# bbc/turingcodec

Hardware: AMD Instinct MI355X
Metric: encoded fps (havoc hot path, primitive-batch throughput: one picture's primitive calls per frame as whole-frame batches; (higher is better)
Workload: dtype u8; 1 GPU; 1920x1080 8-bit 4:2:0 random-access QP32 speed=medium B-frame, MEASURED call mix of the reference encoder on this clip generator (profiles/r04_reference_call_mi; calls_per_frame=3944815, launches_per_frame=49, pictures_in_flight=2, parallelism=single GPU

## Files before the change

### turingcodec_amd/csrc/kernels_metric.hip

```cpp
#include "common.h"

#include <cstdlib>

namespace havoc_gpu {


template <int S>
__device__ __forceinline__ uint32_t sad_dword(uint32_t a, uint32_t b, uint32_t acc)
{
    if (S == 1) return __builtin_amdgcn_sad_u8(a, b, acc);
    return __builtin_amdgcn_sad_u16(a, b, acc);
}

#ifndef SADL
#define SADL 16
#endif
constexpr int kSadLanes = SADL;
__device__ __forceinline__ int sad_group_sum(int v)
{
    v += __builtin_amdgcn_update_dpp(0, v, 0x111, 0xf, 0xf, true);
    v += __builtin_amdgcn_update_dpp(0, v, 0x112, 0xf, 0xf, true);
    v += __builtin_amdgcn_update_dpp(0, v, 0x114, 0xf, 0xe, true);
    if (kSadLanes == 16) v += __builtin_amdgcn_update_dpp(0, v, 0x118, 0xf, 0xc, true);
    return v;
// ... 99 lines not shown
#pragma unroll
    for (int k = 0; k < WAYS; ++k)
    {
        int t = sad_group_sum((int)acc[k]);
        if (S == 2) t >>= 2;
        if (live && lane == kSadLanes - 1) out[job * WAYS + k] = t;
    }
}

constexpr int kSadWinBytes = 1536;

template <int S, int CB>
__device__ __forceinline__ void sad4_window_strips(const char *src, uint32_t s0, uint32_t ssb, const char *ref, uint32_t a0, uint32_t rsb, const __attribute__((address_space(3))) uint32_t *buf_r,
                                                   __attribute__((address_space(3))) uint32_t *buf_w, int pitchD, int chunks, int lead, const int (&ox)[4], const int (&oy)[4],
                                                   int spready, int rowBytes, int h, int hs, int lane, uint32_t (&acc)[4])
{
    const int wstep = smallDiv(kSadLanes, chunks);
    const int wr0 = smallDiv(lane, chunks), wc = lane - mul24(wr0, chunks);
    const bool copies = wr0 < wstep;
    const int cpr = rowBytes / CB;
    const int rpi = smallDiv(kSadLanes, cpr);
    const int y0 = smallDiv(lane, cpr);
    const int xb = (lane - mul24(y0, cpr)) * CB;
    const bool sums = y0 < rpi;
    int lo[4], sh[4];
#pragma unroll
    for (int k = 0; k < 4; ++k)
    {
        const int bo = lead + ox[k] + xb;
        lo[k] = mul24(y0 + oy[k], pitchD) + (bo >> 2);
        sh[k] = bo & 3;
    }
    const int lstep = mul24(rpi, pitchD);
    const uint32_t gstep = mulu24(wstep, rsb), sstep = mulu24(rpi, ssb);
    const int wlstep = mul24(wstep, pitchD);
    for (int ys = 0; ys < h; ys += hs)
    {
        const int he = min(hs, h - ys), nrows = he + spready;
        if (copies)
        {
            uint32_t g = a0 + mulu24(ys + wr0, rsb) + wc * 16;
            int l = mul24(wr0, pitchD) + wc * 4;
            for (int r = wr0; r < nrows; r += wstep, g += gstep, l += wlstep)
            {
                const u32x4 v = ld16(ref + g);
                buf_w[l] = v.x; buf_w[l + 1] = v.y; buf_w[l + 2] = v.z; buf_w[l + 3] = v.w;
            }
        }
        __builtin_amdgcn_fence(__ATOMIC_RELEASE, "wavefront");
        __builtin_amdgcn_wave_barrier();
        __builtin_amdgcn_fence(__ATOMIC_ACQUIRE, "wavefront");
        if (sums)
        {
            uint32_t sp = s0 + mulu24(ys + y0, ssb) + xb;
            int l = 0;
#pragma unroll 2
            for (int y = y0; y < he; y += rpi, sp += sstep, l += lstep)
            {
                if (CB == 16)
                {
                    const u32x4 a = ld16(src + sp);
#pragma unroll
                    for (int k = 0; k < 4; ++k)
                    {
                        const auto q = buf_r + lo[k] + l;
                        const uint32_t d0 = q[0], d1 = q[1], d2 = q[2], d3 = q[3], d4 = q[4];
                        acc[k] = sad_dword<S>(a.x, __builtin_amdgcn_alignbyte(d1, d0, sh[k]), acc[k]);
                        acc[k] = sad_dword<S>(a.y, __builtin_amdgcn_alignbyte(d2, d1, sh[k]), acc[k]);
                        acc[k] = sad_dword<S>(a.z, __builtin_amdgcn_alignbyte(d3, d2, sh[k]), acc[k]);
                        acc[k] = sad_dword<S>(a.w, __builtin_amdgcn_alignbyte(d4, d3, sh[k]), acc[k]);
                    }
                }
                else if (CB == 8)
                {
                    const u32x2 a = ld8(src + sp);
#pragma unroll
                    for (int k = 0; k < 4; ++k)
                    {
                        const auto q = buf_r + lo[k] + l;
                        const uint32_t d0 = q[0], d1 = q[1], d2 = q[2];
                        acc[k] = sad_dword<S>(a.x, __builtin_amdgcn_alignbyte(d1, d0, sh[k]), acc[k]);
                        acc[k] = sad_dword<S>(a.y, __builtin_amdgcn_alignbyte(d2, d1, sh[k]), acc[k]);
                    }
                }
                else
                {
                    const uint32_t a = ld4(src + sp);
#pragma unroll
                    for (int k = 0; k < 4; ++k)
                    {
                        const auto q = buf_r + lo[k] + l;
                        acc[k] = sad_dword<S>(a, __builtin_amdgcn_alignbyte(q[1], q[0], sh[k]), acc[k]);
                    }
                }
            }
        }
        __builtin_amdgcn_fence(__ATOMIC_RELEASE, "wavefront");
        __builtin_amdgcn_wave_barrier();
    }
}

template <int S, int WB>
__device__ __forceinline__ void sad4_job(const char *__restrict__ src, long stride_src, const char *__restrict__ ref, long stride_ref, float inv_stride_ref,
                                         const int32_t *__restrict__ j, bool live, uint32_t *gbuf, int lane, int (&total)[4])
{
    const int so = j[0], w = j[5], h = live ? j[6] : 0;
    int ro[4];
#pragma unroll
    for (int k = 0; k < 4; ++k) ro[k] = j[1 + k];
    const long ssb = stride_src * S, rsb = stride_ref * S;
    const char *s = src + (long)so * S;
    uint32_t acc[4] = {0, 0, 0, 0};
    const int rowBytes = w * S;

    int dx[4] = {0, 0, 0, 0}, dy[4] = {0, 0, 0, 0};
    const int st = (int)stride_ref, half = st >> 1;
#pragma unroll
    for (int k = 1; k < 4; ++k)
    {
        const int delta = ro[k] - ro[0];
        int q = (int)floorf(((float)delta + (float)half) * inv_stride_ref);
        int r = delta - q * st;
        if (r < -half) { --q; r += st; }
        if (r >= st - half) { ++q; r -= st; }
        dx[k] = r; dy[k] = q;
    }
    const int mindx = min(min(dx[0], dx[1]), min(dx[2], dx[3])), maxdx = max(max(dx[0], dx[1]), max(dx[2], dx[3]));
    const int mindy = min(min(dy[0], dy[1]), min(dy[2], dy[3])), maxdy = max(max(dy[0], dy[1]), max(dy[2], dy[3]));
    const int spready = maxdy - mindy;
    const long minoff = ((long)ro[0] + mul24(mindy, st) + mindx) * S;
    const int lead = (int)(reinterpret_cast<uintptr_t>(ref + minoff) & 15);
    const int chunks = (lead + rowBytes + (maxdx - mindx) * S + 15) >> 4;
    const int pitchD = 4 * chunks + 1;
    const int fit = chunks > 0 && chunks <= kSadLanes ? smallDiv(WB * S / 4, pitchD) - spready : 0;
    const bool chunked = (rowBytes & 15) == 0 ? rowBytes <= 16 * kSadLanes : (rowBytes & 7) == 0 ? rowBytes <= 8 * kSadLanes : (rowBytes & 3) == 0 && rowBytes <= 4 * kSadLanes;
    const bool rows24 = (unsigned)spready < 1024u && (unsigned)h <= 64u && ssb < (1 << 23);
    const bool near = rows24 && minoff + (long)mulu24(h + spready, (uint32_t)rsb) + 16 * chunks < (1ll << 32) && ((long)so * S + (long)mulu24(h, (uint32_t)ssb) + rowBytes) < (1ll << 32);
    const bool window = live && chunked && chunks <= kSadLanes && minoff >= 16 && fit >= min(h, 4) && fit >= 1 && near;
    if (window)
    {
        int ox[4], oy[4];
#pragma unroll
        for (int k = 0; k < 4; ++k)
        {
            ox[k] = (dx[k] - mindx) * S;
            oy[k] = dy[k] - mindy;
        }
        const uint32_t a0 = (uint32_t)(minoff - lead), s0 = (uint32_t)so * S;
        const auto buf_r = (const __attribute__((address_space(3))) uint32_t *)(gbuf);
        const auto buf_w = (__attribute__((address_space(3))) uint32_t *)(gbuf);
        const int hs = min(fit, h);
        if ((rowBytes & 15) == 0) sad4_window_strips<S, 16>(src, s0, (uint32_t)ssb, ref, a0, (uint32_t)rsb, buf_r, buf_w, pitchD, chunks, lead, ox, oy, spready, rowBytes, h, hs, lane, acc);
        else if ((rowBytes & 7) == 0) sad4_window_strips<S, 8>(src, s0, (uint32_t)ssb, ref, a0, (uint32_t)rsb, buf_r, buf_w, pitchD, chunks, lead, ox, oy, spready, rowBytes, h, hs, lane, acc);
        else sad4_window_strips<S, 4>(src, s0, (uint32_t)ssb, ref, a0, (uint32_t)rsb, buf_r, buf_w, pitchD, chunks, lead, ox, oy, spready, rowBytes, h, hs, lane, acc);
    }
    else
    {
        typedef typename Sample<S>::T T;
        const char *r[4];
#pragma unroll
        for (int k = 0; k < 4; ++k) r[k] = ref + (long)ro[k] * S;
        if ((rowBytes & 15) == 0 && rowBytes <= 16 * kSadLanes) sad_block<S, 4, 16, 1>(s, ssb, r, rsb, rowBytes, h, lane, acc);
        else if ((rowBytes & 7) == 0 && rowBytes <= 8 * kSadLanes) sad_block<S, 4, 8, 1>(s, ssb, r, rsb, rowBytes, h, lane, acc);
        else if ((rowBytes & 3) == 0 && rowBytes <= 4 * kSadLanes) sad_block<S, 4, 4, 1>(s, ssb, r, rsb, rowBytes, h, lane, acc);
        else
        {
            const FastDiv fd(w);
            for (int i = lane; i < w * h; i += kSadLanes)
            {
                const int y = fd.div(i), x = i - y * w;
                const int a = reinterpret_cast<const T *>(s + y * ssb)[x];
#pragma unroll
                for (int k = 0; k < 4; ++k) acc[k] += abs(a - (int)reinterpret_cast<const T *>(r[k] + y * rsb)[x]);
            }
        }
    }
#pragma unroll
    for (int k = 0; k < 4; ++k)
    {
        int t = sad_group_sum((int)acc[k]);
        if (S == 2) t >>= 2;
        total[k] = t;
    }
}

template <int S, int WB = kSadWinBytes, int MINW = 1>
__global__ __launch_bounds__(256, MINW) void k_sad4w(const char *__restrict__ src, long stride_src, const char *__restrict__ ref, long stride_ref, float inv_stride_ref,
                                               const int32_t *__restrict__ jobs, int njobs, int32_t *__restrict__ out)
{
    constexpr int kBufD = WB * S / 4 + 16;
    __shared__ uint32_t lds[(256 / kSadLanes) * kBufD + 4];
    const int group = threadIdx.x / kSadLanes, lane = threadIdx.x & (kSadLanes - 1);
    const int job = xcd_block(blockIdx.x, gridDim.x) * (256 / kSadLanes) + group;
    const bool live = job < njobs;
    int total[4];
    sad4_job<S, WB>(src, stride_src, ref, stride_ref, inv_stride_ref, jobs + (long)(live ? job : 0) * 8, live, &lds[group * kBufD], lane, total);
    if (live && lane == kSadLanes - 1)
#pragma unroll
        for (int k = 0; k < 4; ++k) out[job * 4 + k] = total[k];
}

constexpr int kRunMax = 128;

template <int S, int CB, int U>
__device__ __forceinline__ void sad4_run_calls(const __attribute__((address_space(3))) uint32_t *win, const __attribute__((address_space(3))) uint32_t *srcw,
                                               const __attribute__((address_space(3))) uint32_t *cand, int pitchD, int lead, int mndx, int mndy, int rowBytes, int h,
                                               int count, int group, int ngroups, int lane, int32_t *__restrict__ out)
{
    const int cpr = rowBytes / CB;
    const int rpi = smallDiv(kSadLanes, cpr);
    const int y0 = smallDiv(lane, cpr);
    const int xb = (lane - mul24(y0, cpr)) * CB;
    const bool sums = y0 < rpi;
    const int lstep = mul24(rpi, pitchD);
    const int s0 = (mul24(y0, rowBytes) + xb) >> 2, sstep = mul24(rpi, rowBytes) >> 2;
    const int base = lead + xb - mndx * S;
    for (int c0 = group; c0 < count; c0 += ngroups * U)
    {
        int lo[4 * U], sh[4 * U];
        uint32_t acc[4 * U];
#pragma unroll
        for (int u = 0; u < U; ++u)
        {
            const int c = min(c0 + u * ngroups, count - 1);
            uint32_t v4[4];
            if (true)
            {
                const u32x4 cv = *reinterpret_cast<const __attribute__((address_space(3))) u32x4 *>(cand + 4 * c);
                v4[0] = cv.x; v4[1] = cv.y; v4[2] = cv.z; v4[3] = cv.w;
            }
#pragma unroll
            for (int k = 0; k < 4; ++k)
            {
                const int v = (int)v4[k];
                const int dx = (int)(short)(v & 0xffff), dy = v >> 16;
                const int bo = base + dx * S;
                lo[4 * u + k] = mul24(y0 + dy - mndy, pitchD) + (bo >> 2);
                sh[4 * u + k] = bo & 3;
                acc[4 * u + k] = 0;
            }
        }
        if (sums)
        {
            int l = 0, sp = s0;
#pragma unroll 2
            for (int y = y0; y < h; y += rpi, sp += sstep, l += lstep)
            {
                if (CB == 16)
                {
                    const u32x4 av = *reinterpret_cast<const __attribute__((address_space(3))) u32x4 *>(srcw + sp);
#pragma unroll
                    for (int k = 0; k < 4 * U; ++k)
                    {
                        const auto q = win + lo[k] + l;
                        const uint32_t d0 = q[0], d1 = q[1], d2 = q[2], d3 = q[3], d4 = q[4];
                        acc[k] = sad_dword<S>(av.x, __builtin_amdgcn_alignbyte(d1, d0, sh[k]), acc[k]);
                        acc[k] = sad_dword<S>(av.y, __builtin_amdgcn_alignbyte(d2, d1, sh[k]), acc[k]);
                        acc[k] = sad_dword<S>(av.z, __builtin_amdgcn_alignbyte(d3, d2, sh[k]), acc[k]);
                        acc[k] = sad_dword<S>(av.w, __builtin_amdgcn_alignbyte(d4, d3, sh[k]), acc[k]);
                    }
                }
                else if (CB == 8)
                {
                    const u32x2 av = *reinterpret_cast<const __attribute__((address_space(3))) u32x2 *>(srcw + sp);
#pragma unroll
                    for (int k = 0; k < 4 * U; ++k)
                    {
                        const auto q = win + lo[k] + l;
                        const uint32_t d0 = q[0], d1 = q[1], d2 = q[2];
                        acc[k] = sad_dword<S>(av.x, __builtin_amdgcn_alignbyte(d1, d0, sh[k]), acc[k]);
                        acc[k] = sad_dword<S>(av.y, __builtin_amdgcn_alignbyte(d2, d1, sh[k]), acc[k]);
                    }
                }
                else
                {
                    const uint32_t a0 = srcw[sp];
#pragma unroll
                    for (int k = 0; k < 4 * U; ++k)
                    {
                        const auto q = win + lo[k] + l;
                        acc[k] = sad_dword<S>(a0, __builtin_amdgcn_alignbyte(q[1], q[0], sh[k]), acc[k]);
                    }
                }
            }
        }
#pragma unroll
        for (int u = 0; u < U; ++u)
        {
            const int c = c0 + u * ngroups;
#pragma unroll
            for (int k = 0; k < 4; ++k)
            {
                int t = sad_group_sum((int)acc[4 * u + k]);
                if (S == 2) t >>= 2;
                if (lane == kSadLanes - 1 && c < count) out[4 * c + k] = t;
            }
        }
    }
}

typedef u32x4 __attribute__((aligned(4))) u32x4_dw;
typedef u32x2 __attribute__((aligned(4))) u32x2_dw;

template <int S, int ND, bool SG>
__device__ __forceinline__ uint32_t sad_lane_rows(const __attribute__((address_space(3))) uint32_t *q, const __attribute__((address_space(3))) uint32_t *s, int pitchD,
                                                  int nd, int rows, int sh, const uint32_t *__restrict__ gs, int gpitch)
{
    uint32_t acc = 0;
    if (SG)
    {
        if (ND >= 4)
        {
            uint32_t a1 = 0, a2 = 0, a3 = 0;
#pragma unroll 2
            for (int y = 0; y < rows; ++y, q += pitchD, gs += gpitch)
            {
                uint32_t prev = q[0];
#pragma unroll
                for (int i = 0; i < ND; i += 4)
                {
                    const u32x4 a = *reinterpret_cast<const u32x4_dw *>(gs + i);
                    const uint32_t d1 = q[i + 1], d2 = q[i + 2], d3 = q[i + 3], d4 = q[i + 4];
                    acc = sad_dword<S>(a.x, __builtin_amdgcn_alignbyte(d1, prev, sh), acc);
                    a1 = sad_dword<S>(a.y, __builtin_amdgcn_alignbyte(d2, d1, sh), a1);
                    a2 = sad_dword<S>(a.z, __builtin_amdgcn_alignbyte(d3, d2, sh), a2);
                    a3 = sad_dword<S>(a.w, __builtin_amdgcn_alignbyte(d4, d3, sh), a3);
                    prev = d4;
                }
            }
            acc += a1 + a2 + a3;
        }
        else if (ND == 2)
        {
#pragma unroll 4
            for (int y = 0; y < rows; ++y, q += pitchD, gs += gpitch)
            {
                const u32x2 a = *reinterpret_cast<const u32x2_dw *>(gs);
                const uint32_t d0 = q[0], d1 = q[1], d2 = q[2];
                acc = sad_dword<S>(a.x, __builtin_amdgcn_alignbyte(d1, d0, sh), acc);
                acc = sad_dword<S>(a.y, __builtin_amdgcn_alignbyte(d2, d1, sh), acc);
            }
        }
        else
        {
            for (int y = 0; y < rows; ++y, q += pitchD, gs += gpitch)
            {
                uint32_t prev = q[0];
                for (int i = 0; i < nd; ++i)
                {
                    const uint32_t d = q[i + 1];
                    acc = sad_dword<S>(gs[i], __builtin_amdgcn_alignbyte(d, prev, sh), acc);
                    prev = d;
                }
            }
        }
        return acc;
    }
    if (ND >= 4)
    {
#pragma unroll 2
        for (int y = 0; y < rows; ++y, q += pitchD, s += ND)
        {
            uint32_t prev = q[0];
#pragma unroll
            for (int i = 0; i < ND; i += 4)
            {
                const u32x4 a = *reinterpret_cast<const __attribute__((address_space(3))) u32x4 *>(s + i);
                const uint32_t d1 = q[i + 1], d2 = q[i + 2], d3 = q[i + 3], d4 = q[i + 4];
                acc = sad_dword<S>(a.x, __builtin_amdgcn_alignbyte(d1, prev, sh), acc);
                acc = sad_dword<S>(a.y, __builtin_amdgcn_alignbyte(d2, d1, sh), acc);
                acc = sad_dword<S>(a.z, __builtin_amdgcn_alignbyte(d3, d2, sh), acc);
                acc = sad_dword<S>(a.w, __builtin_amdgcn_alignbyte(d4, d3, sh), acc);
                prev = d4;
            }
        }
    }
    else if (ND == 2)
    {
#pragma unroll 4
        for (int y = 0; y < rows; ++y, q += pitchD, s += 2)
        {
            const u32x2 a = *reinterpret_cast<const __attribute__((address_space(3))) u32x2 *>(s);
            const uint32_t d0 = q[0], d1 = q[1], d2 = q[2];
            acc = sad_dword<S>(a.x, __builtin_amdgcn_alignbyte(d1, d0, sh), acc);
            acc = sad_dword<S>(a.y, __builtin_amdgcn_alignbyte(d2, d1, sh), acc);
        }
    }
    else
    {
        for (int y = 0; y < rows; ++y, q += pitchD, s += nd)
        {
            uint32_t prev = q[0];
            for (int i = 0; i < nd; ++i)
            {
                const uint32_t d = q[i + 1];
                acc = sad_dword<S>(s[i], __builtin_amdgcn_alignbyte(d, prev, sh), acc);
                prev = d;
            }
        }
    }
    return acc;
}

template <int S, int NW, bool SG>
__device__ __forceinline__ void sad4_run_lanes(const __attribute__((address_space(3))) uint32_t *win, const __attribute__((address_space(3))) uint32_t *srcw,
                                               const __attribute__((address_space(3))) uint32_t *cand, uint32_t *s_acc, int pitchD, int lead, int mndx,
                                               int mndy, int rowBytes, int h, int count, int tid, int32_t *__restrict__ out, const uint32_t *__restrict__ gsrc, int gpitch)
{
    const int P = 4 * count, nd = rowBytes >> 2, chunks = (P + 63) >> 6;
    const int wave = __builtin_amdgcn_readfirstlane(tid >> 6), lane = tid & 63;
    int ns = 1;
    while (ns < 8 && chunks * ns < NW && h >= 16 * ns) ns *= 2;
    const int rps = (h + ns - 1) / ns;
    if (ns > 1)
    {
        for (int i = tid; i < P; i += 64 * NW) s_acc[i] = 0;
        __syncthreads();
    }
    for (int t = wave; t < chunks * ns; t += NW)
    {
        const int chunk = ns == 1 ? t : t / ns, slice = t - chunk * ns;
        const int pos = chunk * 64 + lane;
        const int p = pos;
        const int v = (int)cand[min(p, P - 1)];
        const int col = (int)(short)(v & 0xffff) - mndx, row = (v >> 16) - mndy;
        const int bo = lead + col * S, sh = bo & 3;
        const int yBeg = slice * rps, rows = min(h, yBeg + rps) - yBeg;
        const auto q = win + mul24(row + yBeg, pitchD) + (bo >> 2);
        const auto sp = srcw + yBeg * nd;
        const uint32_t *gs = gsrc + (long)yBeg * gpitch;
        uint32_t acc;
        if (S == 2 && nd == 32) acc = sad_lane_rows<S, 32, SG>(q, sp, pitchD, nd, rows, sh, gs, gpitch);
        else if (nd == 16) acc = sad_lane_rows<S, 16, SG>(q, sp, pitchD, nd, rows, sh, gs, gpitch);
        else if (nd == 8) acc = sad_lane_rows<S, 8, SG>(q, sp, pitchD, nd, rows, sh, gs, gpitch);
        else if (nd == 4) acc = sad_lane_rows<S, 4, SG>(q, sp, pitchD, nd, rows, sh, gs, gpitch);
        else if (nd == 2) acc = sad_lane_rows<S, 2, SG>(q, sp, pitchD, nd, rows, sh, gs, gpitch);
        else acc = sad_lane_rows<S, 0, SG>(q, sp, pitchD, nd, rows, sh, gs, gpitch);
        if (p < P)
        {
            if (ns == 1) out[p] = (int32_t)(S == 2 ? acc >> 2 : acc);
            else atomicAdd(&s_acc[p], acc);
        }
    }
    if (ns > 1)
    {
        __syncthreads();
        for (int p = tid; p < P; p += 64 * NW) out[p] = (int32_t)(S == 2 ? s_acc[p] >> 2 : s_acc[p]);
    }
}

template <int S>
struct RunLds
{
    static constexpr int kWinD = (S == 1 ? 16 : 32) * 256;
    static constexpr int kSrcD = 64 * 64 * S / 4;
    __attribute__((aligned(16))) uint32_t lds[kWinD + kSrcD + 8];
    __attribute__((aligned(16))) uint32_t cand[kRunMax * 4];
    uint32_t acc[kRunMax * 4];
    int box[6];
};

template <int S, int NW, int U, bool SRCG>
__device__ __forceinline__ void sad4_run_general(RunLds<S> &sh, const char *__restrict__ src, long stride_src, const char *__restrict__ ref, long stride_ref,
                                                 float inv_stride_ref, const int32_t *__restrict__ jobs, int njobs, const int32_t *__restrict__ runs, int run,
                                                 int32_t *__restrict__ out)
{
    constexpr int T = 64 * NW, NG = T / kSadLanes;
    constexpr int kWinD = RunLds<S>::kWinD, kSrcD = RunLds<S>::kSrcD;
    constexpr int kFallWB = 1024, kFallD = kFallWB * S / 4 + 16;
    static_assert(NG * kFallD + 4 <= kWinD + kSrcD, "the call-by-call path's buffers must fit the run's LDS");
    uint32_t (&lds)[kWinD + kSrcD + 8] = sh.lds;
    uint32_t (&s_cand)[kRunMax * 4] = sh.cand;
    uint32_t (&s_acc)[kRunMax * 4] = sh.acc;
    int (&s_box)[6] = sh.box;
    const int tid = threadIdx.x, lane = tid & (kSadLanes - 1), group = tid / kSadLanes;
    const int32_t *rr = runs + (long)run * 8;
    const int first = rr[0], count = rr[1], boxOff = rr[2], boxW = rr[3], boxH = rr[4];
    if (first < 0 || count <= 0 || (long)first + count > njobs) return;
    const int32_t *j0 = jobs + (long)first * 8;
    const int so = j0[0], ro0 = j0[1], w = j0[5], h = j0[6];
    const int st = (int)stride_ref, half = st >> 1;
    const int rowBytes = w * S;
    const long ssb = stride_src * S, rsb = stride_ref * S;
    const bool chunked = (rowBytes & 15) == 0 ? rowBytes <= 16 * kSadLanes : (rowBytes & 7) == 0 ? rowBytes <= 8 * kSadLanes : (rowBytes & 3) == 0 && rowBytes <= 4 * kSadLanes;
    const bool srcScalar = U == 0 && SRCG && (((reinterpret_cast<uintptr_t>(src) + (long)so * S) | ssb) & 3) == 0;
    const bool given = boxW > 0 && boxH > 0 && boxW < st;
    int mndx = 0, mndy = 0, spanx, spready, ok = count <= kRunMax;
    long minoff;
    if (given)
    {
        spanx = boxW - w;
        spready = boxH - h;
        minoff = (long)boxOff * S;
        ok &= spanx >= 0 && spready >= 0 && boxOff >= 0;
    }
    else
    {
        if (tid < 6) s_box[tid] = tid == 4 ? 1 : 0;
        __syncthreads();
        int mn_x = 0, mx_x = 0, mn_y = 0, mx_y = 0;
        for (int p = tid; p < 4 * min(count, kRunMax); p += T)
        {
            const int32_t *j = j0 + (p >> 2) * 8;
            const int delta = j[1 + (p & 3)] - ro0;
            int q = (int)floorf(((float)delta + (float)half) * inv_stride_ref);
            long rl = (long)delta - (long)q * st;
            if (rl < -half) { --q; rl += st; }
            if (rl >= st - half) { ++q; rl -= st; }
            ok &= (j[0] == so) & (j[5] == w) & (j[6] == h) & (q >= -32768) & (q < 32768) & (rl >= -32768) & (rl < 32768);
            const int r = (int)rl;
            s_cand[p] = (uint32_t)(r & 0xffff) | ((uint32_t)q << 16);
            mn_x = min(mn_x, r); mx_x = max(mx_x, r); mn_y = min(mn_y, q); mx_y = max(mx_y, q);
        }
#pragma unroll
        for (int o = 1; o < 64; o <<= 1)
        {
            mn_x = min(mn_x, __shfl_xor(mn_x, o, 64)); mx_x = max(mx_x, __shfl_xor(mx_x, o, 64));
            mn_y = min(mn_y, __shfl_xor(mn_y, o, 64)); mx_y = max(mx_y, __shfl_xor(mx_y, o, 64));
            ok &= __shfl_xor(ok, o, 64);
        }
        if ((tid & 63) == 0)
        {
            atomicMin(&s_box[0], mn_x); atomicMax(&s_box[1], mx_x); atomicMin(&s_box[2], mn_y); atomicMax(&s_box[3], mx_y); atomicAnd(&s_box[4], ok);
        }
        __syncthreads();
        mndx = s_box[0];
        mndy = s_box[2];
        spanx = s_box[1] - mndx;
        spready = s_box[3] - mndy;
        ok = s_box[4];
        minoff = ((long)ro0 + (long)mndy * st + mndx) * S;
    }
    const int lead = (int)(reinterpret_cast<uintptr_t>(ref + minoff) & 15);
    const int chunks = (lead + rowBytes + spanx * S + 15) >> 4;
    const int pitchD = 4 * chunks + 1, rows = h + spready;
    const bool near = (unsigned)spready < 1024u && (unsigned)h <= 64u && ssb < (1 << 23) && rsb < (1 << 23) && chunks <= 1024 && spanx >= 0 &&
                      minoff + (long)rows * rsb + 16l * chunks < (1ll << 32) && ((long)so * S + (long)h * ssb + rowBytes) < (1ll << 32);
    bool fits = ok && chunked && near && w <= 64 && minoff >= 16 && (long)pitchD * rows + 4 <= kWinD;
    if (fits)
    {
        const auto win_w = (__attribute__((address_space(3))) uint32_t *)(&lds[0]);
        const auto src_w = (__attribute__((address_space(3))) uint32_t *)(&lds[kWinD + 4]);
        {
            const FastDiv fc(chunks);
            const uint32_t a0 = (uint32_t)(minoff - lead);
            for (int i = tid; i < rows * chunks; i += T)
            {
                const int r = fc.div(i), c = i - r * chunks;
                const u32x4 v = ld16(ref + a0 + (uint32_t)r * (uint32_t)rsb + c * 16);
                const int l = r * pitchD + c * 4;
                win_w[l] = v.x; win_w[l + 1] = v.y; win_w[l + 2] = v.z; win_w[l + 3] = v.w;
            }
            if (!srcScalar)
            {
                const int dpr = rowBytes >> 2;
                const FastDiv fdw(dpr);
                const uint32_t sb0 = (uint32_t)so * S;
                for (int i = tid; i < h * dpr; i += T)
                {
                    const int y = fdw.div(i), x = i - y * dpr;
                    src_w[i] = ld4(src + sb0 + (uint32_t)y * (uint32_t)ssb + x * 4);
                }
            }
        }
        if (given)
        {
            int in = 1;
            for (int p = tid; p < 4 * count; p += T)
            {
                const int32_t *j = j0 + (p >> 2) * 8;
                const int delta = j[1 + (p & 3)] - boxOff;
                int q = (int)(((float)delta + 0.5f) * inv_stride_ref);
                int r = delta - q * st;
                if (r < 0) { --q; r += st; }
                if (r >= st) { ++q; r -= st; }
                in &= (j[0] == so) & (j[5] == w) & (j[6] == h) & (delta >= 0) & (q >= 0) & (q <= spready) & (r >= 0) & (r <= spanx);
                s_cand[p] = (uint32_t)(r & 0xffff) | ((uint32_t)q << 16);
            }
            fits = __syncthreads_and(in) != 0;
        }
        else
            __syncthreads();
    }
    if (fits)
    {
        const auto win = (const __attribute__((address_space(3))) uint32_t *)(&lds[0]);
        const auto srcw = (const __attribute__((address_space(3))) uint32_t *)(&lds[kWinD + 4]);
        const auto cand = (const __attribute__((address_space(3))) uint32_t *)(&s_cand[0]);
        int32_t *o = out + (long)first * 4;
        if (U == 0)
        {
            const long sbyte = (long)so * S;
            if (srcScalar)
                sad4_run_lanes<S, NW, true>(win, srcw, cand, s_acc, pitchD, lead, mndx, mndy, rowBytes, h, count, tid, o, reinterpret_cast<const uint32_t *>(src + sbyte), (int)(ssb >> 2));
            else
                sad4_run_lanes<S, NW, false>(win, srcw, cand, s_acc, pitchD, lead, mndx, mndy, rowBytes, h, count, tid, o, nullptr, 0);
        }
        else if ((rowBytes & 15) == 0) sad4_run_calls<S, 16, (U ? U : 1)>(win, srcw, cand, pitchD, lead, mndx, mndy, rowBytes, h, count, group, NG, lane, o);
        else if ((rowBytes & 7) == 0) sad4_run_calls<S, 8, (U ? U : 1)>(win, srcw, cand, pitchD, lead, mndx, mndy, rowBytes, h, count, group, NG, lane, o);
        else sad4_run_calls<S, 4, (U ? U : 1)>(win, srcw, cand, pitchD, lead, mndx, mndy, rowBytes, h, count, group, NG, lane, o);
        return;
    }
    __syncthreads();
    for (int c = group; c < ((count + NG - 1) / NG) * NG; c += NG)
    {
        const bool live = c < count;
        int total[4];
        sad4_job<S, kFallWB>(src, stride_src, ref, stride_ref, inv_stride_ref, j0 + (long)(live ? c : 0) * 8, live, &lds[group * kFallD], lane, total);
        if (live && lane == kSadLanes - 1)
#pragma unroll
            for (int k = 0; k < 4; ++k) out[((long)first + c) * 4 + k] = total[k];
    }
}

template <int S, int NW, int U, bool SRCG = true>
__global__ __launch_bounds__(64 * NW) void k_sad4r(const char *__restrict__ src, long stride_src, const char *__restrict__ ref, long stride_ref, float inv_stride_ref,
                                                   const int32_t *__restrict__ jobs, int njobs, const int32_t *__restrict__ runs, int nruns, int32_t *__restrict__ out)
{
    __shared__ RunLds<S> sh;
    sad4_run_general<S, NW, U, SRCG>(sh, src, stride_src, ref, stride_ref, inv_stride_ref, jobs, njobs, runs, xcd_block(blockIdx.x, gridDim.x), out);
}


template <int S>
__device__ __forceinline__ uint32_t ssd_dword(uint32_t a, uint32_t b, uint32_t acc)
{
    if (S == 1)
    {
        acc = __builtin_amdgcn_udot4(a, a, acc, false);
        acc = __builtin_amdgcn_udot4(b, b, acc, false);
        const uint32_t ab = __builtin_amdgcn_udot4(a, b, 0u, false);
        return acc - 2u * ab;
    }
    const u16x2 va = __builtin_bit_cast(u16x2, a), vb = __builtin_bit_cast(u16x2, b);
    acc = __builtin_amdgcn_udot2(va, va, acc, false);
    acc = __builtin_amdgcn_udot2(vb, vb, acc, false);
    const uint32_t ab = __builtin_amdgcn_udot2(va, vb, 0u, false);
    return acc - 2u * ab;
}

template <int S, int CB>
__device__ __forceinline__ uint32_t ssd_block(const char *a, long sab, const char *b, long sbb, int rowBytes, int h, int lane)
{
    const int cpr = rowBytes / CB;
    const int rpi = kSadLanes / cpr;
    const int y0 = lane / cpr;
    const int xb = (lane - y0 * cpr) * CB;
    uint32_t acc = 0;
    if (y0 >= rpi) return 0;
#pragma unroll 2
    for (int y = y0; y < h; y += rpi)
    {
        const char *p = a + y * sab + xb, *q = b + y * sbb + xb;
        if (CB == 4) acc = ssd_dword<S>(ld4(p), ld4(q), acc);
        else if (CB == 8)
        {
            const u32x2 u = ld8(p), v = ld8(q);
            acc = ssd_dword<S>(u.x, v.x, acc);
            acc = ssd_dword<S>(u.y, v.y, acc);
        }
        else
        {
            const u32x4 u = ld16(p), v = ld16(q);
            acc = ssd_dword<S>(u.x, v.x, acc);
            acc = ssd_dword<S>(u.y, v.y, acc);
            acc = ssd_dword<S>(u.z, v.z, acc);
            acc = ssd_dword<S>(u.w, v.w, acc);
        }
    }
    return acc;
}

template <int S>
__global__ __launch_bounds__(256) void k_ssd(const char *__restrict__ pa, long stride_a, const char *__restrict__ pb, long stride_b,
                                             const int32_t *__restrict__ jobs, int njobs, uint32_t *__restrict__ out)
{
    typedef typename Sample<S>::T T;
    const int job = (xcd_block(blockIdx.x, gridDim.x) * 256 + threadIdx.x) / kSadLanes;
    const int lane = threadIdx.x & (kSadLanes - 1);
    const bool live = job < njobs;
    const int32_t *j = jobs + (long)(live ? job : 0) * 4;
    const int w = j[2], h = live ? j[3] : 0;
    const long sab = stride_a * S, sbb = stride_b * S;
    const char *a = pa + (long)j[0] * S;
    const char *b = pb + (long)j[1] * S;
    uint32_t acc = 0;
    const int rowBytes = w * S;
    if ((rowBytes & 15) == 0 && rowBytes <= 16 * kSadLanes) acc = ssd_block<S, 16>(a, sab, b, sbb, rowBytes, h, lane);
    else if ((rowBytes & 7) == 0 && rowBytes <= 8 * kSadLanes) acc = ssd_block<S, 8>(a, sab, b, sbb, rowBytes, h, lane);
    else if ((rowBytes & 3) == 0 && rowBytes <= 4 * kSadLanes) acc = ssd_block<S, 4>(a, sab, b, sbb, rowBytes, h, lane);
    else
    {
        const FastDiv fd(w);
        for (int i = lane; i < w * h; i += kSadLanes)
        {
            const int y = fd.div(i), x = i - y * w;
            const int d = (int)reinterpret_cast<const T *>(a + y * sab)[x] - (int)reinterpret_cast<const T *>(b + y * sbb)[x];
            acc += (uint32_t)(d * d);
        }
    }
    uint32_t t = (uint32_t)sad_group_sum((int)acc);
    if (S == 2) t >>= 4;
    if (live && lane == kSadLanes - 1) out[job] = t;
}


template <int S, int N>
__device__ __forceinline__ void load_diff_row(const char *a, const char *b, int (&d)[N])
{
    if (S == 1)
    {
        if (N == 8)
        {
            const u32x2 va = ld8(a), vb = ld8(b);
#pragma unroll
            for (int x = 0; x < 4; ++x)
            {
                d[x] = (int)((va.x >> (8 * x)) & 0xff) - (int)((vb.x >> (8 * x)) & 0xff);
                d[x + 4] = (int)((va.y >> (8 * x)) & 0xff) - (int)((vb.y >> (8 * x)) & 0xff);
            }
        }
        else
        {
            const uint32_t va = ld4(a), vb = ld4(b);
#pragma unroll
            for (int x = 0; x < 4; ++x) d[x] = (int)((va >> (8 * x)) & 0xff) - (int)((vb >> (8 * x)) & 0xff);
        }
    }
    else
    {
        if (N == 8)
        {
            const u32x4 va = ld16(a), vb = ld16(b);
            const uint32_t wa[4] = {va.x, va.y, va.z, va.w}, wb[4] = {vb.x, vb.y, vb.z, vb.w};
#pragma unroll
            for (int x = 0; x < 4; ++x)
            {
                d[2 * x] = (int)(wa[x] & 0xffff) - (int)(wb[x] & 0xffff);
                d[2 * x + 1] = (int)(wa[x] >> 16) - (int)(wb[x] >> 16);
            }
        }
        else
        {
            const u32x2 va = ld8(a), vb = ld8(b);
            d[0] = (int)(va.x & 0xffff) - (int)(vb.x & 0xffff);
            d[1] = (int)(va.x >> 16) - (int)(vb.x >> 16);
            d[2] = (int)(va.y & 0xffff) - (int)(vb.y & 0xffff);
            d[3] = (int)(va.y >> 16) - (int)(vb.y >> 16);
        }
    }
}

template <int S, int G>
__global__ __launch_bounds__(256) void k_satd(const char *__restrict__ pa, long stride_a, const char *__restrict__ pb, long stride_b,
                                              const int32_t *__restrict__ jobs, int njobs, int32_t *__restrict__ out)
{
    typedef typename Sample<S>::T T;
    const int job = (xcd_block(blockIdx.x, gridDim.x) * 256 + threadIdx.x) / G;
    const int l = threadIdx.x & (G - 1);
    const bool live = job < njobs;
    const int32_t *j = jobs + (long)(live ? job : 0) * 4;
    const int w = j[2], h = live ? j[3] : 0;
    const long sab = stride_a * S, sbb = stride_b * S;
    const char *a = pa + (long)j[0] * S;
    const char *b = pb + (long)j[1] * S;
    int acc = 0;
    if (((w | h) & 7) == 0)
    {
        const int tw = w >> 3;
        const FastDiv fd(tw);
        for (int it = l; it < tw * (h >> 3) * 8; it += G)
        {
            const int tile = it >> 3, r = it & 7;
            const int ty = fd.div(tile), tx = tile - ty * tw;
            const char *pa8 = a + (long)(ty * 8 + r) * sab + tx * 8 * S, *pb8 = b + (long)(ty * 8 + r) * sbb + tx * 8 * S;
            if (S == 1)
            {
                const u32x2 va = ld8(pa8), vb = ld8(pb8);
                const uint32_t m = 0x00ff00ffu;
                uint32_t p[4] = {pk_sub(va.x & m, vb.x & m), pk_sub((va.x >> 8) & m, (vb.x >> 8) & m),
                                 pk_sub(va.y & m, vb.y & m), pk_sub((va.y >> 8) & m, (vb.y >> 8) & m)};
                acc += satd_rows_pk<8>(p, r);
            }
            else
            {
                int d[8];
                load_diff_row<S, 8>(pa8, pb8, d);
                acc += satd_rows<S, 8>(d, r);
            }
        }
    }
    else if (((w | h) & 3) == 0)
    {
        const int tw = w >> 2;
        const FastDiv fd(tw);
        for (int it = l; it < tw * (h >> 2) * 4; it += G)
        {
            const int tile = it >> 2, r = it & 3;
            const int ty = fd.div(tile), tx = tile - ty * tw;
            const char *pa4 = a + (long)(ty * 4 + r) * sab + tx * 4 * S, *pb4 = b + (long)(ty * 4 + r) * sbb + tx * 4 * S;
            if (S == 1)
            {
                const uint32_t va = ld4(pa4), vb = ld4(pb4), m = 0x00ff00ffu;
                uint32_t p[2] = {pk_sub(va & m, vb & m), pk_sub((va >> 8) & m, (vb >> 8) & m)};
                acc += satd_rows_pk<4>(p, r);
            }
            else
            {
                int d[4];
                load_diff_row<S, 4>(pa4, pb4, d);
                acc += satd_rows<S, 4>(d, r);
            }
        }
    }
    else
    {
        const int tw = w >> 1;
        const FastDiv fd(tw);
        for (int t = l; t < tw * (h >> 1); t += G)
        {
            const int ty = fd.div(t), tx = t - ty * tw;
            const T *p = reinterpret_cast<const T *>(a + (long)(2 * ty) * sab) + 2 * tx;
            const T *q = reinterpret_cast<const T *>(b + (long)(2 * ty) * sbb) + 2 * tx;
            const int d0 = (int)p[0] - (int)q[0], d1 = (int)p[1] - (int)q[1];
            const int d2 = (int)p[stride_a] - (int)q[stride_b], d3 = (int)p[stride_a + 1] - (int)q[stride_b + 1];
            int sum = abs(d0 + d1 + d2 + d3) + abs(d0 - d1 + d2 - d3) + abs(d0 + d1 - d2 - d3) + abs(d0 - d1 - d2 + d3);
            if (S == 2) sum >>= 2;
            acc += sum;
        }
    }
    const int t = G == 64 ? wave_sum(acc) : group_sum<G>(acc);
    if (live && l == 0) out[job] = t;
}

constexpr int kSatdMulti = 16;

template <int S, int G, int CPS, bool TILE = false>
__global__ __launch_bounds__(256) void k_satd_multi(const char *__restrict__ pa, long stride_a, const char *__restrict__ pb, long stride_b,
                                                    const int32_t *__restrict__ jobs, int njobs, int32_t *__restrict__ out)
{
    typedef typename Sample<S>::T T;
    constexpr int SL = kSatdMulti / CPS;
    const int grp = (xcd_block(blockIdx.x, gridDim.x) * 256 + threadIdx.x) / G;
    const int job = grp / SL, k0 = (grp - job * SL) * CPS;
    const int l = threadIdx.x & (G - 1);
    const bool live = job < njobs;
    const int32_t *j = jobs + (long)(live ? job : 0) * (4 + kSatdMulti);
    const int w = j[1], cnt = min(max(j[3], 0), kSatdMulti), h = (live && k0 < cnt) ? j[2] : 0;
    const long sab = stride_a * S, sbb = stride_b * S;
    const char *a = pa + (long)j[0] * S;
    const char *b[CPS];
#pragma unroll
    for (int k = 0; k < CPS; ++k) b[k] = pb + (long)j[4 + max(0, min(k0 + k, cnt - 1))] * S;
    int acc[CPS];
#pragma unroll
    for (int k = 0; k < CPS; ++k) acc[k] = 0;
    if (TILE && S == 2 && ((w | h) & 7) == 0)
    {
        const int tw = w >> 3;
        const FastDiv fd(tw);
        for (int t = l; t < tw * (h >> 3); t += G)
        {
            const int ty = fd.div(t), tx = t - ty * tw;
            const char *pa8 = a + (long)(ty * 8) * sab + tx * 16;
            const long ob = (long)(ty * 8) * sbb + tx * 16;
            uint32_t ap[8][4];
#pragma unroll
            for (int r = 0; r < 8; ++r)
            {
                const u32x4 va = ld16(pa8 + r * sab);
                ap[r][0] = va.x; ap[r][1] = va.y; ap[r][2] = va.z; ap[r][3] = va.w;
            }
#pragma unroll
            for (int k = 0; k < CPS; ++k)
            {
                uint32_t d[8][4];
#pragma unroll
                for (int r = 0; r < 8; ++r)
                {
                    const u32x4 vb = ld16(b[k] + ob + r * sbb);
                    d[r][0] = pk_sub(ap[r][0], vb.x); d[r][1] = pk_sub(ap[r][1], vb.y); d[r][2] = pk_sub(ap[r][2], vb.z); d[r][3] = pk_sub(ap[r][3], vb.w);
                }
                acc[k] += satd_tile8_pk16(d);
            }
        }
    }
    else if (TILE && S == 1 && ((w | h) & 7) == 0)
    {
        const int tw = w >> 3;
        const FastDiv fd(tw);
        const uint32_t m = 0x00ff00ffu;
        for (int t = l; t < tw * (h >> 3); t += G)
        {
            const int ty = fd.div(t), tx = t - ty * tw;
            const char *pa8 = a + (long)(ty * 8) * sab + tx * 8;
            const long ob = (long)(ty * 8) * sbb + tx * 8;
            uint32_t ap[8][4];
#pragma unroll
            for (int r = 0; r < 8; ++r)
            {
                const u32x2 va = ld8(pa8 + r * sab);
                ap[r][0] = va.x & m; ap[r][1] = (va.x >> 8) & m; ap[r][2] = va.y & m; ap[r][3] = (va.y >> 8) & m;
            }
#pragma unroll
// ... 263 lines not shown
```

Baseline: 1547 frames/s.

## Prefetch source rows into a register ring ahead of SAD loop in lanes path

When the source block is read straight from global memory in the per-lane SAD4 run path, rows are now loaded into a small register ring several rows ahead. The first fill is issued before the window staging and candidate check, so the global source loads overlap LDS staging and the barrier rather than stalling inside the SAD loop. This costs extra VGPRs for the ring and adds control logic for wraparound, slicing and tail rows, which could lower occupancy or add branch overhead.

```diff
diff --git a/turingcodec_amd/csrc/kernels_metric.hip b/turingcodec_amd/csrc/kernels_metric.hip
--- a/turingcodec_amd/csrc/kernels_metric.hip
+++ b/turingcodec_amd/csrc/kernels_metric.hip
@@ -425,60 +425,158 @@
 typedef u32x4 __attribute__((aligned(4))) u32x4_dw;
 typedef u32x2 __attribute__((aligned(4))) u32x2_dw;
 
-template <int S, int ND, bool SG>
-__device__ __forceinline__ uint32_t sad_lane_rows(const __attribute__((address_space(3))) uint32_t *q, const __attribute__((address_space(3))) uint32_t *s, int pitchD,
-                                                  int nd, int rows, int sh, const uint32_t *__restrict__ gs, int gpitch)
-{
+#ifndef HAVOC_SAD4_SRC_DIST
+#define HAVOC_SAD4_SRC_DIST 4
+#endif
+#ifndef HAVOC_SAD4_SRC_RING
+#define HAVOC_SAD4_SRC_RING 4
+#endif
+constexpr int kSrcRingQ = HAVOC_SAD4_SRC_RING;
+template <int ND> struct SrcDist { static constexpr int D = ND == 0 ? 8 : 4 * kSrcRingQ <= ND ? 1 : 4 * kSrcRingQ / ND < HAVOC_SAD4_SRC_DIST ? 4 * kSrcRingQ / ND : HAVOC_SAD4_SRC_DIST; };
+static_assert(HAVOC_SAD4_SRC_DIST >= 1 && HAVOC_SAD4_SRC_DIST <= kSrcRingQ, "the narrow rows' distance must fit the ring");
+template <int ND>
+struct SrcRing
+{
+    static constexpr int N = ND >= 4 ? SrcDist<ND>::D * ND / 4 : ND == 2 ? SrcDist<ND>::D : SrcDist<ND>::D / 4;
+    u32x4 v[N];
+    int beg;
+};
+
+template <int ND>
+__device__ __forceinline__ void src_ring_fill(SrcRing<ND> &r, const uint32_t *__restrict__ gs, int gpitch, int nd, int rows)
+{
+    constexpr int D = SrcDist<ND>::D;
+    if (ND >= 4)
+    {
+#pragma unroll
+        for (int k = 0; k < D; ++k)
+        {
+            const uint32_t *g = gs + (long)(k < rows ? k : 0) * gpitch;
+#pragma unroll
+            for (int j = 0; j < ND / 4; ++j) r.v[k * (ND / 4) + j] = *reinterpret_cast<const u32x4_dw *>(g + 4 * j);
+        }
+    }
+    else if (ND == 2)
+    {
+#pragma unroll
+        for (int k = 0; k < D; ++k)
+        {
+            const u32x2 a = *reinterpret_cast<const u32x2_dw *>(gs + (long)(k < rows ? k : 0) * gpitch);
+            r.v[k].x = a.x; r.v[k].y = a.y;
+        }
+    }
+    else
+    {
+        int col = 0, row = 0;
+        const uint32_t *g = gs;
+#pragma unroll
+        for (int k = 0; k < D; ++k)
+        {
+            r.v[k >> 2][k & 3] = g[col];
+            if (++col == nd) { col = 0; g += gpitch; if (++row == rows) { row = 0; g = gs; } }
+        }
+    }
+}
+
+template <int S, int ND>
+__device__ __forceinline__ uint32_t sad_lane_rows_ring(const __attribute__((address_space(3))) uint32_t *q, int pitchD, int nd, int rows, int sh, SrcRing<ND> &r,
+                                                       const uint32_t *__restrict__ gs, int gpitch)
+{
+    constexpr int D = SrcDist<ND>::D;
     uint32_t acc = 0;
-    if (SG)
-    {
-        if (ND >= 4)
-        {
-            uint32_t a1 = 0, a2 = 0, a3 = 0;
-#pragma unroll 2
-            for (int y = 0; y < rows; ++y, q += pitchD, gs += gpitch)
+    if (ND != 0)
+    {
+        constexpr int NP = ND >= 4 ? ND / 4 : 1;
+        uint32_t a1 = 0, a2 = 0, a3 = 0;
+        auto row = [&](int k, const uint32_t *gn, bool load) __attribute__((always_inline)) {
+            if (ND >= 4)
             {
                 uint32_t prev = q[0];
 #pragma unroll
                 for (int i = 0; i < ND; i += 4)
                 {
-                    const u32x4 a = *reinterpret_cast<const u32x4_dw *>(gs + i);
+                    const u32x4 a = r.v[k * NP + i / 4];
                     const uint32_t d1 = q[i + 1], d2 = q[i + 2], d3 = q[i + 3], d4 = q[i + 4];
                     acc = sad_dword<S>(a.x, __builtin_amdgcn_alignbyte(d1, prev, sh), acc);
                     a1 = sad_dword<S>(a.y, __builtin_amdgcn_alignbyte(d2, d1, sh), a1);
                     a2 = sad_dword<S>(a.z, __builtin_amdgcn_alignbyte(d3, d2, sh), a2);
                     a3 = sad_dword<S>(a.w, __builtin_amdgcn_alignbyte(d4, d3, sh), a3);
+                    if (load) r.v[k * NP + i / 4] = *reinterpret_cast<const u32x4_dw *>(gn + i);
                     prev = d4;
                 }
             }
-            acc += a1 + a2 + a3;
-        }
-        else if (ND == 2)
-        {
-#pragma unroll 4
-            for (int y = 0; y < rows; ++y, q += pitchD, gs += gpitch)
-            {
-                const u32x2 a = *reinterpret_cast<const u32x2_dw *>(gs);
+            else
+            {
                 const uint32_t d0 = q[0], d1 = q[1], d2 = q[2];
-                acc = sad_dword<S>(a.x, __builtin_amdgcn_alignbyte(d1, d0, sh), acc);
-                acc = sad_dword<S>(a.y, __builtin_amdgcn_alignbyte(d2, d1, sh), acc);
-            }
-        }
-        else
-        {
-            for (int y = 0; y < rows; ++y, q += pitchD, gs += gpitch)
-            {
-                uint32_t prev = q[0];
-                for (int i = 0; i < nd; ++i)
+                acc = sad_dword<S>(r.v[k].x, __builtin_amdgcn_alignbyte(d1, d0, sh), acc);
+                a1 = sad_dword<S>(r.v[k].y, __builtin_amdgcn_alignbyte(d2, d1, sh), a1);
+                if (load)
                 {
-                    const uint32_t d = q[i + 1];
-                    acc = sad_dword<S>(gs[i], __builtin_amdgcn_alignbyte(d, prev, sh), acc);
-                    prev = d;
+                    const u32x2 a = *reinterpret_cast<const u32x2_dw *>(gn);
+                    r.v[k].x = a.x; r.v[k].y = a.y;
                 }
             }
-        }
-        return acc;
-    }
+            q += pitchD;
+        };
+        int y = 0, nrow = D;
+        const uint32_t *gn = gs + (long)D * gpitch;
+        for (; y + D <= rows; y += D)
+        {
+#pragma unroll
+            for (int k = 0; k < D; ++k)
+            {
+                if (nrow >= rows) { nrow = 0; gn = gs; }
+                row(k, gn, true);
+                ++nrow;
+                gn += gpitch;
+            }
+        }
+        if (y < rows)
+        {
+#pragma unroll
+            for (int k = 0; k < D - 1; ++k)
+                if (y + k < rows) row(k, gs, false);
+            if (y != 0) r.beg = -1;
+        }
+        return acc + a1 + a2 + a3;
+    }
+    const int total = rows * nd;
+    int col = 0, prow = 0, pcol = 0, e = 0;
+    const uint32_t *gn = gs;
+#pragma unroll
+    for (int k = 0; k < D; ++k)
+        if (++pcol == nd) { pcol = 0; gn += gpitch; if (++prow == rows) { prow = 0; gn = gs; } }
+    uint32_t prev = 0;
+    auto dword = [&](int k, bool load) __attribute__((always_inline)) {
+        if (col == 0) prev = q[0];
+        const uint32_t d = q[col + 1];
+        acc = sad_dword<S>(r.v[k >> 2][k & 3], __builtin_amdgcn_alignbyte(d, prev, sh), acc);
+        prev = d;
+        if (load)
+        {
+            r.v[k >> 2][k & 3] = gn[pcol];
+            if (++pcol == nd) { pcol = 0; gn += gpitch; if (++prow == rows) { prow = 0; gn = gs; } }
+        }
+        if (++col == nd) { col = 0; q += pitchD; }
+    };
+    for (; e + D <= total; e += D)
+#pragma unroll
+        for (int k = 0; k < D; ++k) dword(k, true);
+    if (e < total)
+    {
+#pragma unroll
+        for (int k = 0; k < D - 1; ++k)
+            if (e + k < total) dword(k, false);
+        if (e != 0) r.beg = -1;
+    }
+    return acc;
+}
+
+template <int S, int ND>
+__device__ __forceinline__ uint32_t sad_lane_rows(const __attribute__((address_space(3))) uint32_t *q, const __attribute__((address_space(3))) uint32_t *s, int pitchD,
+                                                  int nd, int rows, int sh)
+{
+    uint32_t acc = 0;
     if (ND >= 4)
     {
 #pragma unroll 2
@@ -525,15 +623,22 @@
     return acc;
 }
 
-template <int S, int NW, bool SG>
+template <int NW>
+__device__ __forceinline__ int sad4_lane_slices(int chunks, int h)
+{
+    int ns = 1;
+    while (ns < 8 && chunks * ns < NW && h >= 16 * ns) ns *= 2;
+    return ns;
+}
+
+template <int S, int NW>
 __device__ __forceinline__ void sad4_run_lanes(const __attribute__((address_space(3))) uint32_t *win, const __attribute__((address_space(3))) uint32_t *srcw,
                                                const __attribute__((address_space(3))) uint32_t *cand, uint32_t *s_acc, int pitchD, int lead, int mndx,
-                                               int mndy, int rowBytes, int h, int count, int tid, int32_t *__restrict__ out, const uint32_t *__restrict__ gsrc, int gpitch)
+                                               int mndy, int rowBytes, int h, int count, int tid, int32_t *__restrict__ out)
 {
     const int P = 4 * count, nd = rowBytes >> 2, chunks = (P + 63) >> 6;
     const int wave = __builtin_amdgcn_readfirstlane(tid >> 6), lane = tid & 63;
-    int ns = 1;
-    while (ns < 8 && chunks * ns < NW && h >= 16 * ns) ns *= 2;
+    const int ns = sad4_lane_slices<NW>(chunks, h);
     const int rps = (h + ns - 1) / ns;
     if (ns > 1)
     {
@@ -551,14 +656,13 @@
         const int yBeg = slice * rps, rows = min(h, yBeg + rps) - yBeg;
         const auto q = win + mul24(row + yBeg, pitchD) + (bo >> 2);
         const auto sp = srcw + yBeg * nd;
-        const uint32_t *gs = gsrc + (long)yBeg * gpitch;
         uint32_t acc;
-        if (S == 2 && nd == 32) acc = sad_lane_rows<S, 32, SG>(q, sp, pitchD, nd, rows, sh, gs, gpitch);
-        else if (nd == 16) acc = sad_lane_rows<S, 16, SG>(q, sp, pitchD, nd, rows, sh, gs, gpitch);
-        else if (nd == 8) acc = sad_lane_rows<S, 8, SG>(q, sp, pitchD, nd, rows, sh, gs, gpitch);
-        else if (nd == 4) acc = sad_lane_rows<S, 4, SG>(q, sp, pitchD, nd, rows, sh, gs, gpitch);
-        else if (nd == 2) acc = sad_lane_rows<S, 2, SG>(q, sp, pitchD, nd, rows, sh, gs, gpitch);
-        else acc = sad_lane_rows<S, 0, SG>(q, sp, pitchD, nd, rows, sh, gs, gpitch);
+        if (S == 2 && nd == 32) acc = sad_lane_rows<S, 32>(q, sp, pitchD, nd, rows, sh);
+        else if (nd == 16) acc = sad_lane_rows<S, 16>(q, sp, pitchD, nd, rows, sh);
+        else if (nd == 8) acc = sad_lane_rows<S, 8>(q, sp, pitchD, nd, rows, sh);
+        else if (nd == 4) acc = sad_lane_rows<S, 4>(q, sp, pitchD, nd, rows, sh);
+        else if (nd == 2) acc = sad_lane_rows<S, 2>(q, sp, pitchD, nd, rows, sh);
+        else acc = sad_lane_rows<S, 0>(q, sp, pitchD, nd, rows, sh);
         if (p < P)
         {
             if (ns == 1) out[p] = (int32_t)(S == 2 ? acc >> 2 : acc);
@@ -570,6 +674,61 @@
         __syncthreads();
         for (int p = tid; p < P; p += 64 * NW) out[p] = (int32_t)(S == 2 ? s_acc[p] >> 2 : s_acc[p]);
     }
+}
+
+template <int S, int NW, int ND, typename Staged>
+__device__ __forceinline__ bool sad4_run_lanes_ring(Staged &&staged, const __attribute__((address_space(3))) uint32_t *win,
+                                                    const __attribute__((address_space(3))) uint32_t *cand, uint32_t *s_acc, int pitchD, int lead, int mndx, int mndy,
+                                                    int rowBytes, int h, int count, int tid, int32_t *__restrict__ out, const uint32_t *__restrict__ gsrc, int gpitch)
+{
+    const int P = 4 * count, nd = rowBytes >> 2, chunks = (P + 63) >> 6;
+    const int wave = __builtin_amdgcn_readfirstlane(tid >> 6), lane = tid & 63;
+    const int ns = sad4_lane_slices<NW>(chunks, h);
+    const int rps = (h + ns - 1) / ns;
+    SrcRing<ND> ring;
+    ring.beg = -1;
+    if (wave < chunks * ns)
+    {
+        const int chunk = ns == 1 ? wave : wave / ns, slice = wave - chunk * ns;
+        const int yBeg = slice * rps;
+        src_ring_fill<ND>(ring, gsrc + (long)yBeg * gpitch, gpitch, nd, min(h, yBeg + rps) - yBeg);
+        ring.beg = yBeg;
+    }
+    if (!staged()) return false;
+    __builtin_amdgcn_s_waitcnt(0x0f70);
+    if (ns > 1)
+    {
+        for (int i = tid; i < P; i += 64 * NW) s_acc[i] = 0;
+        __syncthreads();
+    }
+    for (int t = wave; t < chunks * ns; t += NW)
+    {
+        const int chunk = ns == 1 ? t : t / ns, slice = t - chunk * ns;
+        const int p = chunk * 64 + lane;
+        const int v = (int)cand[min(p, P - 1)];
+        const int col = (int)(short)(v & 0xffff) - mndx, row = (v >> 16) - mndy;
+        const int bo = lead + col * S, sh = bo & 3;
+        const int yBeg = slice * rps, rows = min(h, yBeg + rps) - yBeg;
+        const auto q = win + mul24(row + yBeg, pitchD) + (bo >> 2);
+        const uint32_t *gs = gsrc + (long)yBeg * gpitch;
+        if (ring.beg != yBeg)
+        {
+            src_ring_fill<ND>(ring, gs, gpitch, nd, rows);
+            ring.beg = yBeg;
+        }
+        const uint32_t acc = sad_lane_rows_ring<S, ND>(q, pitchD, nd, rows, sh, ring, gs, gpitch);
+        if (p < P)
+        {
+            if (ns == 1) out[p] = (int32_t)(S == 2 ? acc >> 2 : acc);
+            else atomicAdd(&s_acc[p], acc);
+        }
+    }
+    if (ns > 1)
+    {
+        __syncthreads();
+        for (int p = tid; p < P; p += 64 * NW) out[p] = (int32_t)(S == 2 ? s_acc[p] >> 2 : s_acc[p]);
+    }
+    return true;
 }
 
 template <int S>
@@ -606,7 +765,7 @@
     const int rowBytes = w * S;
     const long ssb = stride_src * S, rsb = stride_ref * S;
     const bool chunked = (rowBytes & 15) == 0 ? rowBytes <= 16 * kSadLanes : (rowBytes & 7) == 0 ? rowBytes <= 8 * kSadLanes : (rowBytes & 3) == 0 && rowBytes <= 4 * kSadLanes;
-    const bool srcScalar = U == 0 && SRCG && (((reinterpret_cast<uintptr_t>(src) + (long)so * S) | ssb) & 3) == 0;
+    const bool srcGlobal = U == 0 && SRCG && (((reinterpret_cast<uintptr_t>(src) + (long)so * S) | ssb) & 3) == 0;
     const bool given = boxW > 0 && boxH > 0 && boxW < st;
     int mndx = 0, mndy = 0, spanx, spready, ok = count <= kRunMax;
     long minoff;
@@ -674,7 +833,7 @@
                 const int l = r * pitchD + c * 4;
                 win_w[l] = v.x; win_w[l + 1] = v.y; win_w[l + 2] = v.z; win_w[l + 3] = v.w;
             }
-            if (!srcScalar)
+            if (!srcGlobal)
             {
                 const int dpr = rowBytes >> 2;
                 const FastDiv fdw(dpr);
@@ -686,8 +845,12 @@
                 }
             }
         }
-        if (given)
-        {
+        auto staged = [&]() __attribute__((always_inline)) -> bool {
+            if (!given)
+            {
+                __syncthreads();
+                return true;
+            }
             int in = 1;
             for (int p = tid; p < 4 * count; p += T)
             {
@@ -700,29 +863,30 @@
                 in &= (j[0] == so) & (j[5] == w) & (j[6] == h) & (delta >= 0) & (q >= 0) & (q <= spready) & (r >= 0) & (r <= spanx);
                 s_cand[p] = (uint32_t)(r & 0xffff) | ((uint32_t)q << 16);
             }
-            fits = __syncthreads_and(in) != 0;
-        }
-        else
-            __syncthreads();
-    }
-    if (fits)
-    {
+            return __syncthreads_and(in) != 0;
+        };
         const auto win = (const __attribute__((address_space(3))) uint32_t *)(&lds[0]);
         const auto srcw = (const __attribute__((address_space(3))) uint32_t *)(&lds[kWinD + 4]);
         const auto cand = (const __attribute__((address_space(3))) uint32_t *)(&s_cand[0]);
         int32_t *o = out + (long)first * 4;
-        if (U == 0)
-        {
-            const long sbyte = (long)so * S;
-            if (srcScalar)
-                sad4_run_lanes<S, NW, true>(win, srcw, cand, s_acc, pitchD, lead, mndx, mndy, rowBytes, h, count, tid, o, reinterpret_cast<const uint32_t *>(src + sbyte), (int)(ssb >> 2));
-            else
-                sad4_run_lanes<S, NW, false>(win, srcw, cand, s_acc, pitchD, lead, mndx, mndy, rowBytes, h, count, tid, o, nullptr, 0);
-        }
-        else if ((rowBytes & 15) == 0) sad4_run_calls<S, 16, (U ? U : 1)>(win, srcw, cand, pitchD, lead, mndx, mndy, rowBytes, h, count, group, NG, lane, o);
-        else if ((rowBytes & 7) == 0) sad4_run_calls<S, 8, (U ? U : 1)>(win, srcw, cand, pitchD, lead, mndx, mndy, rowBytes, h, count, group, NG, lane, o);
-        else sad4_run_calls<S, 4, (U ? U : 1)>(win, srcw, cand, pitchD, lead, mndx, mndy, rowBytes, h, count, group, NG, lane, o);
-        return;
+        if (srcGlobal)
+        {
+            const uint32_t *gsrc = reinterpret_cast<const uint32_t *>(src + (long)so * S);
+            const int gpitch = (int)(ssb >> 2), nd = rowBytes >> 2;
+#define HAVOC_LANES(ND) sad4_run_lanes_ring<S, NW, ND>(staged, win, cand, s_acc, pitchD, lead, mndx, mndy, rowBytes, h, count, tid, o, gsrc, gpitch)
+            if (S == 2 && nd == 32 ? HAVOC_LANES(32) : nd == 16 ? HAVOC_LANES(16) : nd == 8 ? HAVOC_LANES(8) : nd == 4 ? HAVOC_LANES(4) : nd == 2 ? HAVOC_LANES(2) : HAVOC_LANES(0))
+                return;
+#undef HAVOC_LANES
+            fits = false;
+        }
+        else if ((fits = staged()))
+        {
+            if (U == 0) sad4_run_lanes<S, NW>(win, srcw, cand, s_acc, pitchD, lead, mndx, mndy, rowBytes, h, count, tid, o);
+            else if ((rowBytes & 15) == 0) sad4_run_calls<S, 16, (U ? U : 1)>(win, srcw, cand, pitchD, lead, mndx, mndy, rowBytes, h, count, group, NG, lane, o);
+            else if ((rowBytes & 7) == 0) sad4_run_calls<S, 8, (U ? U : 1)>(win, srcw, cand, pitchD, lead, mndx, mndy, rowBytes, h, count, group, NG, lane, o);
+            else sad4_run_calls<S, 4, (U ? U : 1)>(win, srcw, cand, pitchD, lead, mndx, mndy, rowBytes, h, count, group, NG, lane, o);
+            return;
+        }
     }
     __syncthreads();
     for (int c = group; c < ((count + NG - 1) / NG) * NG; c += NG)
```

After: 1545 frames/s. Within noise of the previous version (-0.1%).
